# epam/ai-dial-rag

Measured on AMD Instinct MI355X. Metric: retrieval_qps_10Mx384, higher is better.
Workload: dtype f32 (int8 MFMA filter with exact integer dot products and a rigorous error margin, every candidate the margin cannot exclude re-scored in f64 with the reference formula)

## Files before the change

### ai-dial-rag_amd/csrc/vec_kernels_i8.h

```cpp
#pragma once
#include "vec_kernels_sieve.h"

#ifndef I8_ABL
#define I8_ABL 0
#endif

namespace mir {

typedef int __attribute__((ext_vector_type(4))) i32x4;

constexpr int kI8StatWords = 8;
constexpr int kI8MaxK = 16;
static_assert(kI8MaxK <= kSieveSampleMaxK, "the exact sample threshold evaluates k rows in one round");
constexpr int kI8Region = 32768;
constexpr int kI8WavePart = kI8Region / 8;
__device__ __forceinline__ void i8_margin_ab(float qn, float eq, const float *__restrict__ stats, float &A, float &B) {
    i8_margin_ab_decl(qn, eq, stats, A, B);
}
__device__ __forceinline__ float i8_margin_tile(bool l2, float A, float B, float e_t, float s_t, float sq) {
    const float m = fmaf(e_t, A, B) + 2.0f * s_t * sq;
    return l2 ? 2.0f * m : m;
}

__global__ __launch_bounds__(256) void i8_tile_scale_kernel(const float *__restrict__ src, int64_t n, int d, float4 *__restrict__ tparam) {
    __shared__ float red[4];
    const int64_t tile = blockIdx.x;
    const int64_t r0 = tile * kTileRows;
    const int64_t rows = n - r0 < kTileRows ? n - r0 : kTileRows;
    const float *p = src + r0 * (int64_t)d;
    float m = 0.f;
    for (int64_t i = threadIdx.x; i < rows * d; i += 256) m = fmaxf(m, fabsf(p[i]));
#pragma unroll
    for (int off = 32; off >= 1; off >>= 1) m = fmaxf(m, __shfl_xor(m, off, 64));
    if ((threadIdx.x & 63) == 0) red[threadIdx.x >> 6] = m;
    __syncthreads();
    if (threadIdx.x == 0) {
        m = fmaxf(fmaxf(red[0], red[1]), fmaxf(red[2], red[3]));
        const float st = m > 0.f ? m / 127.0f : 1.0f;
        tparam[tile] = make_float4(st, 0.f, 0.5f / st, 0.f);
    }
}
__global__ void i8_scale_kernel(float *__restrict__ stats, const float *__restrict__ max_norm) {
    stats[0] = max_norm[0];
    stats[7] = __builtin_inff();
}

__device__ __forceinline__ int i8_quant(float x, float inv) {
    const float r = rintf(x * inv);
    return (int)fminf(fmaxf(r, -127.0f), 127.0f);
}

__global__ __launch_bounds__(256) void pack_i8_kernel(const float *__restrict__ src, int64_t n, int d, int ks64, int64_t total_lanes,
                                                      const float4 *__restrict__ tparam, uint4 *__restrict__ dst) {
    const int64_t gid = (int64_t)blockIdx.x * 256 + threadIdx.x;
    if (gid >= total_lanes) return;
    const int lane = (int)(gid & 63);
    const int64_t blk = gid >> 6;
    const int nb = ks64 * 2;
    const int b = (int)(blk % nb);
    const int64_t tile = blk / nb;
    const int s = b >> 1, rh = b & 1;
    const int64_t row = tile * kTileRows + 16 * rh + (lane & 15);
    const int col0 = 64 * s + 16 * (lane >> 4);
    uint32_t w[4] = {0u, 0u, 0u, 0u};
    if (row < n) {
        const float inv = 1.0f / tparam[tile].x;
#pragma unroll
        for (int j = 0; j < 16; ++j) {
            const float x = col0 + j < d ? src[row * (int64_t)d + col0 + j] : 0.f;
            w[j >> 2] |= ((uint32_t)i8_quant(x, inv) & 0xffu) << (8 * (j & 3));
        }
    }
    dst[blk * 64 + lane] = make_uint4(w[0], w[1], w[2], w[3]);
}

__global__ __launch_bounds__(256) void i8_residual_kernel(const float *__restrict__ src, int64_t n, int d, const float *__restrict__ doc_sq,
                                                          float4 *__restrict__ tparam, float *__restrict__ stats) {
    const int lg = threadIdx.x & 15;
    const int64_t row = (int64_t)blockIdx.x * 16 + (threadIdx.x >> 4);
    double e2 = 0.0;
    if (row < n) {
        const float s = tparam[row / kTileRows].x;
        const float inv = 1.0f / s;
        for (int j = lg; j < d; j += 16) {
            const float x = src[row * (int64_t)d + j];
            const double r = (double)x - (double)s * (double)i8_quant(x, inv);
            e2 += r * r;
        }
    }
    e2 = group_sum<16>(e2);
    if (lg == 0 && row < n) {
        const float e = (float)sqrt(e2) * (1.0f + 1e-6f);
        atomicMax(reinterpret_cast<unsigned int *>(&tparam[row / kTileRows].y), __float_as_uint(e));
        const float a = doc_sq[row];
        const volatile float *vs = stats;
        if (e > vs[2]) atomicMax(reinterpret_cast<unsigned int *>(stats) + 2, __float_as_uint(e));
        if (a > vs[1]) atomicMax(reinterpret_cast<unsigned int *>(stats) + 1, __float_as_uint(a));
        if (a < vs[7]) atomicMin(reinterpret_cast<unsigned int *>(stats) + 7, __float_as_uint(a));
    }
}

__global__ __launch_bounds__(128) void i8_stage_record_kernel(const float *__restrict__ col, int64_t n_col, const float4 *__restrict__ tparam,
                                                              float *__restrict__ rec) {
    const int64_t stage = blockIdx.x;
    const int t = threadIdx.x;
    if (t >= 72) return;
    float v;
    if (t < 64) {
        const int64_t row = stage * 64 + t;
        v = row < n_col ? col[row] : 0.f;
    } else {
        v = reinterpret_cast<const float *>(tparam)[stage * 8 + (t - 64)];
    }
    rec[stage * 72 + t] = v;
}

__global__ __launch_bounds__(64) void prep_queries_i8_stats_kernel(const double *__restrict__ q, int b, int d, double *__restrict__ q_sq,
                                                                   double *__restrict__ q_norm, float *__restrict__ q_amax,
                                                                   unsigned long long *__restrict__ gthr, int gthr_words) {
    const int lane = threadIdx.x, blk = blockIdx.x;
    if (gthr && blk * 64 + lane < gthr_words) gthr[blk * 64 + lane] = 0;
    const int qi = blk;
    if (qi >= b) return;
    double s = 0.0;
    float m = 0.f;
    bool bad = false;
    for (int j = lane; j < d; j += 64) {
        const double x = q[(int64_t)qi * d + j];
        s += x * x;
        const float a = fabsf((float)x);
        bad |= !(a < __builtin_inff());
        m = fmaxf(m, a);
    }
    s = wave_sum(s);
#pragma unroll
    for (int off = 32; off >= 1; off >>= 1) m = fmaxf(m, __shfl_xor(m, off, 64));
    bad = __any(bad);
    if (lane == 0) {
        q_sq[qi] = s;
        q_norm[qi] = sqrt(s);
        q_amax[qi] = bad ? -1.0f : m;
    }
}
__global__ __launch_bounds__(64) void prep_queries_i8_quant_kernel(const double *__restrict__ q, int b, int d, int ks64, int ntiles16,
                                                                   const float *__restrict__ q_amax, uint4 *__restrict__ qfrag,
                                                                   double *__restrict__ q_err, float *__restrict__ q_scale) {
    const int lane = threadIdx.x, blk = blockIdx.x;
    if (blk < ntiles16 * ks64) {
        const int s = blk % ks64, w = blk / ks64;
        const int qi = 16 * w + (lane & 15);
        const int col0 = 64 * s + 16 * (lane >> 4);
        uint32_t wv[4] = {0u, 0u, 0u, 0u};
        const float m = qi < b ? q_amax[qi] : -1.0f;
        if (m >= 0.f) {
            const float inv = m > 0.f ? 127.0f / m : 1.0f;
#pragma unroll
            for (int j = 0; j < 16; ++j) {
                const float x = col0 + j < d ? (float)q[(int64_t)qi * d + col0 + j] : 0.f;
                wv[j >> 2] |= ((uint32_t)i8_quant(x, inv) & 0xffu) << (8 * (j & 3));
            }
        }
        qfrag[(int64_t)blk * 64 + lane] = make_uint4(wv[0], wv[1], wv[2], wv[3]);
    } else {
        const int qi = blk - ntiles16 * ks64;
        if (qi >= b) return;
        const float m = q_amax[qi];
        const bool ok = m >= 0.f;
        const float inv = m > 0.f ? 127.0f / m : 1.0f;
        const float sq = 1.0f / inv;
        double e2 = 0.0;
        for (int j = lane; j < d; j += 64) {
            const double x = q[(int64_t)qi * d + j];
            const double r = ok ? x - (double)sq * (double)i8_quant((float)x, inv) : x;
            e2 += r * r;
        }
        e2 = wave_sum(e2);
        if (lane == 0) {
            q_err[qi] = sqrt(e2);
            q_scale[qi] = sq;
        }
    }
}

__host__ __device__ constexpr int sieve_i8_stages(int nw) { return nw == 8 ? kSieveStages : 3; }
__host__ __device__ constexpr size_t sieve_i8_lds_bytes(int ks64, int nw) { return (size_t)sieve_i8_stages(nw) * (ks64 * 4 * 1024 + (64 + 8) * 4) + 64; }

template <int KS64, int KIND, bool SAMPLE, int QT, int NW>
__global__ __launch_bounds__(NW * 64, 2) void sieve_i8_kernel(const uint4 *__restrict__ docs, const float *__restrict__ aux,
                                                          const uint4 *__restrict__ qfrag, const double *__restrict__ q_norm,
                                                          const double *__restrict__ q_sq, const double *__restrict__ q_err,
                                                          const float *__restrict__ stats, const float *__restrict__ q_scale,
                                                          uint32_t n_rows, uint32_t stage0, uint32_t n_stages, int nq, int nan_guard,
                                                          const uint64_t *__restrict__ gthr, uint64_t *__restrict__ cand,
                                                          float *__restrict__ candv, uint32_t *__restrict__ ccount,
                                                          float *__restrict__ part_sample, unsigned long long *__restrict__ stat) {
    static_assert(KIND == SCAN_L2 || KIND == SCAN_IP || KIND == SCAN_COS, "scan kind");
    static_assert(QT == 1 || QT == 2 || QT == 4, "query tiles per wave");
    static_assert(NW == 8 || NW == 4, "waves per workgroup");
    constexpr int NS = sieve_i8_stages(NW);
    constexpr int APW = 64 / NW;
    constexpr int NB = KS64 * 2;
    constexpr int SB = NB * 2;
    constexpr int STAGE_U4 = SB * 64;
    constexpr int PPW = SB / NW;
    constexpr int PW = PPW + 1;
    constexpr int AS = 64 + 8;
    constexpr int D = NS - 1;
    constexpr int QPL = NW * 16 * QT;
    static_assert(SB % NW == 0, "sieve_i8: d padded to a multiple of 128");
    extern __shared__ __attribute__((aligned(16))) unsigned char smem[];
    uint4 *ring = reinterpret_cast<uint4 *>(smem);
    float *aux_lds = reinterpret_cast<float *>(smem + (size_t)NS * STAGE_U4 * 16);

    const int tid = threadIdx.x, lane = tid & 63, qc = lane & 15, jg = lane >> 4;
    const int wave8 = __builtin_amdgcn_readfirstlane(tid >> 6);
    const uint32_t G = gridDim.x;

    const float amin = KIND == SCAN_L2 ? stats[7] : 0.f;
    int qloc[QT];
    bool lane_live[QT];
    unsigned long long live_mask[QT];
    constexpr float L = KIND == SCAN_L2 ? 2.0f : 1.0f;
    const float ax_hi = KIND == SCAN_COS ? stats[6] : 1.0f;
    float tbc[QT];
    float sq[QT], mA[QT], mB[QT], P1[QT], A1[QT], guard[QT], best[QT];
    uint32_t brow[QT];
    i32x4 qh[QT][KS64];
    const bool active = nq > wave8 * QT * 16;
#pragma unroll
    for (int u = 0; u < QT; ++u) {
        const int t16 = wave8 * QT + u;
        qloc[u] = t16 * 16 + qc;
        lane_live[u] = qloc[u] < nq && (SAMPLE || query_filterable(KIND == SCAN_L2, q_norm[qloc[u]], stats[0]));
        live_mask[u] = __builtin_amdgcn_ballot_w64(lane_live[u]);
        sq[u] = 1.0f; mA[u] = 0.f; mB[u] = 0.f; P1[u] = -__builtin_inff(); A1[u] = 0.f; tbc[u] = -__builtin_inff();
        guard[u] = __builtin_inff(); best[u] = -__builtin_inff(); brow[u] = 0;
        if (lane_live[u]) {
            const float qn = (float)q_norm[qloc[u]] * (1.0f + 1e-6f);
            const float eq = (float)q_err[qloc[u]] * (1.0f + 1e-6f);
            const bool good = qn < __builtin_inff() && eq < __builtin_inff();
            sq[u] = q_scale[qloc[u]];
            if (good) i8_margin_ab(qn, eq, stats, mA[u], mB[u]);
            if (!SAMPLE) {
                const uint64_t key = gthr[qloc[u]];
                if (key != 0 && good) {
                    const float t = key_value(key);
                    float tb = t - 2e-6f * fabsf(t);
                    tbc[u] = tb;
                    if (KIND == SCAN_COS) tb = fminf(tb * stats[4], tb * stats[5]) - 1e-6f * fabsf(tb) * stats[5];
                    P1[u] = (tb + amin - L * mB[u]) / (L * sq[u]);
                    A1[u] = mA[u] / sq[u];
                    if (!(P1[u] == P1[u]) || !(A1[u] == A1[u])) { P1[u] = -__builtin_inff(); A1[u] = 0.f; tbc[u] = -__builtin_inff(); }
                }
            } else if (nan_guard) {
                const float qs = (float)q_sq[qloc[u]];
                guard[u] = qs - 1e-5f * fabsf(qs);
            }
        }
        const uint4 *qs = qfrag + (size_t)t16 * KS64 * 64 + lane;
#pragma unroll
        for (int s = 0; s < KS64; ++s) qh[u][s] = __builtin_bit_cast(i32x4, qs[s * 64]);
    }
    const uint32_t my_stages = blockIdx.x < n_stages ? (n_stages - blockIdx.x + G - 1) / G : 0;
    const uint32_t NG = my_stages;

    auto issue = [&](uint32_t g) {
        const uint32_t stage = stage0 + blockIdx.x + g * G;
        const uint4 *src = docs + (size_t)stage * STAGE_U4 + (wave8 * PPW) * 64 + lane;
        const uint32_t dst = __builtin_amdgcn_readfirstlane(lds_addr_of(ring) + ((g % NS) * STAGE_U4 + (wave8 * PPW) * 64) * 16);
#pragma unroll
        for (int i = 0; i < PPW; ++i) glds16_b128(src + i * 64, dst + i * 1024);
        {
            const uint32_t adst = __builtin_amdgcn_readfirstlane(lds_addr_of(aux_lds) + ((g % NS) * AS + wave8 * APW) * 4);
            const float *abase = aux + (size_t)stage * AS + wave8 * APW;
            if (lane < APW + (wave8 == NW - 1 ? 8 : 0)) glds4_b32_sv(abase, (uint32_t)lane * 4u, adst);
        }
    };
#pragma unroll
    for (int u = 0; u < QT; ++u)
#pragma unroll
        for (int s = 0; s < KS64; ++s) asm volatile("" : "+v"(qh[u][s]));
    asm volatile("s_waitcnt vmcnt(0)" ::: "memory");
    for (uint32_t g = 0; g < (uint32_t)D && g < NG; ++g) issue(g);

    auto wait_stage = [&](uint32_t g) {
        const uint32_t younger = (NG - 1 - g) < (uint32_t)(D - 1) ? (NG - 1 - g) : (uint32_t)(D - 1);
        if (younger == (uint32_t)(D - 1)) asm volatile("s_waitcnt vmcnt(%0)" ::"i"((D - 1) * PW) : "memory");
        else asm volatile("s_waitcnt vmcnt(0)" ::: "memory");
    };
    uint64_t *region = cand + ((size_t)blockIdx.x * NW + wave8) * kI8WavePart;
    float *regionv = candv + ((size_t)blockIdx.x * NW + wave8) * kI8WavePart;
    const unsigned long long lt_mask = (1ull << lane) - 1ull;
    uint32_t wcount = 0;

    auto filter = [&](int u, const i32x4 &c0, const i32x4 &c1, const float (&ax)[8], uint32_t t, const float4 &tp) {
        if (SAMPLE) {
            if (lane_live[u]) {
                const float vs = L * tp.x * sq[u], mg = i8_margin_tile(KIND == SCAN_L2, mA[u], mB[u], tp.y, tp.x, sq[u]) * ax_hi;
#pragma unroll
                for (int r = 0; r < 8; ++r) {
                    const float fi = (float)(r < 4 ? c0[r & 3] : c1[r & 3]);
                    const float w = KIND == SCAN_L2 ? fmaf(vs, fi, -ax[r]) : KIND == SCAN_COS ? vs * fi * ax[r] : vs * fi;
                    const uint32_t row = t * kTileRows + 4 * jg + 16 * (r >> 2) + (r & 3);
                    if (w + mg < guard[u] && w - mg > best[u] && row < n_rows) { best[u] = w - mg; brow[u] = row; }
                }
            }
            return;
        }
        const float x2 = fmaf(fmaf(-tp.y, A1[u], P1[u]), 2.0f * tp.z, -4.0f);
        const int ib = (int)__builtin_amdgcn_fmed3f(floorf(x2), -2.0e9f, 2.0e9f);
        const int m0 = max(max(c0[0], c0[1]), c0[2]), m1 = max(max(c0[3], c1[0]), c1[1]);
        const int m = max(max(max(c1[2], c1[3]), m0), m1);
        if ((__builtin_amdgcn_ballot_w64(m >= ib) & live_mask[u]) == 0ull) return;
        asm volatile("" : "+s"(t));
        const float vs = L * tp.x * sq[u];
        float bound = (fmaf(-tp.y, A1[u], P1[u]) - 2.0f * tp.x) * (L * sq[u]) - amin;
        if (KIND == SCAN_COS) bound = tbc[u] - i8_margin_tile(false, mA[u], mB[u], tp.y, tp.x, sq[u]) * ax_hi;
        const float bound_w = bound - 4e-6f * (fabsf(bound) + amin);
        float v[8];
#pragma unroll
        for (int r = 0; r < 8; ++r) {
            const float fi = (float)(r < 4 ? c0[r & 3] : c1[r & 3]);
            v[r] = KIND == SCAN_L2 ? fmaf(vs, fi, -ax[r]) : KIND == SCAN_COS ? vs * fi * ax[r] : vs * fi;
        }
        uint32_t pm = 0;
#pragma unroll
        for (int r = 0; r < 8; ++r) pm |= (uint32_t)(!(v[r] < bound_w)) << r;
        if (!lane_live[u]) pm = 0;
        if (!__any(pm != 0)) return;
        const uint32_t row0 = t * kTileRows + 4 * jg;
        if (t * kTileRows + kTileRows > n_rows) {
#pragma unroll
            for (int r = 0; r < 8; ++r)
                if (row0 + 16 * (r >> 2) + (r & 3) >= n_rows) pm &= ~(1u << r);
        }
        while (__any(pm != 0)) {
            const bool has = pm != 0;
            const int r = has ? __builtin_ctz(pm) : 0;
            const unsigned long long bal = __ballot(has);
            const uint32_t slot = wcount + (uint32_t)__popcll(bal & lt_mask);
            wcount += (uint32_t)__popcll(bal);
            float vr = v[0];
#pragma unroll
            for (int i = 1; i < 8; ++i) vr = r == i ? v[i] : vr;
            if (has && slot < (uint32_t)kI8WavePart) {
                region[slot] = ((uint64_t)(uint32_t)qloc[u] << 32) | (uint64_t)(row0 + 16 * (r >> 2) + (r & 3));
                regionv[slot] = vr;
            }
            pm &= pm - 1;
        }
    };

    i32x4 p0[QT], p1[QT];
#pragma unroll
    for (int u = 0; u < QT; ++u) { p0[u] = i32x4{0, 0, 0, 0}; p1[u] = i32x4{0, 0, 0, 0}; }
    float pax[8] = {};
    float4 ptp = make_float4(1.f, 0.f, 0.5f, 0.f);
    uint32_t pt = 0;
    bool have_prev = false;
    for (uint32_t g = 0; g < my_stages; ++g) {
        const uint32_t stage = stage0 + blockIdx.x + g * G;
#if !(I8_ABL & 4)
        wait_stage(g);
#endif
#if !(I8_ABL & 2)
        __builtin_amdgcn_s_barrier();
#endif
        if (!active) {
            if (g + D < NG) issue(g + D);
            continue;
        }
#pragma unroll
        for (int sub = 0; sub < 2; ++sub) {
            const uint4 *st = ring + (size_t)(g % NS) * STAGE_U4 + sub * (NB * 64) + lane;
            constexpr int PF = QT == 4 ? 1 : (2 < KS64 ? 2 : KS64 - 1);
            uint4 f0[PF + 1], f1[PF + 1];
#pragma unroll
            for (int i = 0; i < PF; ++i) { f0[i] = st[(2 * i + 0) * 64]; f1[i] = st[(2 * i + 1) * 64]; }
            const float4 ctp = *reinterpret_cast<const float4 *>(aux_lds + (g % NS) * AS + 64 + 4 * sub);
            float cax[8] = {};
            if (KIND != SCAN_IP) {
                const float4 a0 = *reinterpret_cast<const float4 *>(aux_lds + (g % NS) * AS + 32 * sub + 4 * jg);
                const float4 a1 = *reinterpret_cast<const float4 *>(aux_lds + (g % NS) * AS + 32 * sub + 16 + 4 * jg);
                cax[0] = a0.x; cax[1] = a0.y; cax[2] = a0.z; cax[3] = a0.w;
                cax[4] = a1.x; cax[5] = a1.y; cax[6] = a1.z; cax[7] = a1.w;
            }
            i32x4 c0[QT], c1[QT];
#pragma unroll
            for (int u = 0; u < QT; ++u) { c0[u] = i32x4{0, 0, 0, 0}; c1[u] = i32x4{0, 0, 0, 0}; }
#pragma unroll
            for (int s = 0; s < KS64; ++s) {
                if (s + PF < KS64) {
                    f0[(s + PF) % (PF + 1)] = st[(2 * (s + PF) + 0) * 64];
                    f1[(s + PF) % (PF + 1)] = st[(2 * (s + PF) + 1) * 64];
                }
                __builtin_amdgcn_sched_barrier(0);
#pragma unroll
                for (int u = 0; u < QT; ++u) {
                    c0[u] = __builtin_amdgcn_mfma_i32_16x16x64_i8(__builtin_bit_cast(i32x4, f0[s % (PF + 1)]), qh[u][s], c0[u], 0, 0, 0);
                    c1[u] = __builtin_amdgcn_mfma_i32_16x16x64_i8(__builtin_bit_cast(i32x4, f1[s % (PF + 1)]), qh[u][s], c1[u], 0, 0, 0);
                }
                if (sub == 0 && s == 0) {
                    __builtin_amdgcn_sched_barrier(0);
#if !(I8_ABL & 4)
                    if (g + D < NG) issue(g + D);
#endif
                }
#pragma unroll
                for (int u = 0; u < QT; ++u)
                    if (s == 1 + u && s < KS64 && have_prev) {
                        __builtin_amdgcn_sched_barrier(0);
#if I8_ABL & 1
                        if (g == 0xffffff)
#endif
                        filter(u, p0[u], p1[u], pax, pt, ptp);
                    }
            }
            if (KS64 < QT + 1 && have_prev) {
#pragma unroll
                for (int u = KS64 - 1; u < QT; ++u) filter(u, p0[u], p1[u], pax, pt, ptp);
            }
#pragma unroll
            for (int u = 0; u < QT; ++u) { p0[u] = c0[u]; p1[u] = c1[u]; }
#pragma unroll
            for (int i = 0; i < 8; ++i) pax[i] = cax[i];
            ptp = ctp;
            pt = stage * 2 + sub;
            have_prev = true;
        }
    }
    if (have_prev) {
#pragma unroll
        for (int u = 0; u < QT; ++u) filter(u, p0[u], p1[u], pax, pt, ptp);
    }
    if (SAMPLE) {
        uint32_t *part_row = reinterpret_cast<uint32_t *>(part_sample + (size_t)gridDim.x * QPL * 2);
#pragma unroll
        for (int u = 0; u < QT; ++u) {
            const float o = __shfl_xor(best[u], 16, 64);
            const uint32_t orow = (uint32_t)__shfl_xor((int)brow[u], 16, 64);
            const bool other = o > best[u];
            const float b2 = other ? o : best[u];
            const size_t at = ((size_t)blockIdx.x * QPL + qloc[u]) * 2 + (jg >> 1);
            if (lane_live[u] && (jg == 0 || jg == 2)) {
                part_sample[at] = b2;
                part_row[at] = other ? orow : brow[u];
            }
        }
        return;
    }
    if (lane == 0) {
        ccount[(size_t)blockIdx.x * NW + wave8] = wcount;
        if (stat && wcount) atomicAdd(stat, (unsigned long long)wcount);
    }
}

__global__ __launch_bounds__(256) void sieve_scatter_i8_kernel(SieveScatterArgs a) {
    __shared__ uint32_t s_cnt[256], s_base[256];
    const int tid = threadIdx.x;
    const int part = blockIdx.x;
    uint32_t cnt = a.ccount[part];
    s_cnt[tid] = 0;
    __syncthreads();
    if (cnt > (uint32_t)kI8WavePart) {
        for (int i = tid; i < a.nq; i += 256) a.l.over[a.q0 + i] = 1;
        cnt = kI8WavePart;
    }
    const uint64_t *region = a.cand + (size_t)part * kI8WavePart;
    const float *regionv = a.candv + (size_t)part * kI8WavePart;
    for (uint32_t e = tid; e < cnt; e += 256) atomicAdd(&s_cnt[(int)(region[e] >> 32) & 255], 1u);
    __syncthreads();
    {
        const uint32_t c = s_cnt[tid];
        s_base[tid] = c ? atomicAdd(&a.l.count[(size_t)(a.q0 + tid) * kSieveCountStride], c) : 0u;
        s_cnt[tid] = 0;
    }
    __syncthreads();
    for (uint32_t e = tid; e < cnt; e += 256) {
        const uint64_t key = region[e];
        const int ql = (int)(key >> 32) & 255, qi = a.q0 + ql;
        const uint32_t slot = s_base[ql] + atomicAdd(&s_cnt[ql], 1u);
        if (slot < (uint32_t)kSieveQueryCap) {
            a.l.row[(size_t)qi * kSieveQueryCap + slot] = (uint32_t)key;
            a.l.rv[(size_t)qi * kSieveQueryCap + slot] = regionv[e];
        } else {
            a.l.over[qi] = 1;
        }
    }
}

}
```

Measured before the change: 254,400.

## Restructure int8 MFMA loop to filter one query tile behind with double-buffered accumulators

The per-stage loop changes from processing two row-halves with QT query accumulators each to iterating over 2*QT query blocks. Each block uses one pair of double-buffered accumulators, and the filter test for the previous block is interleaved inside the MFMA chain. All K fragments of a half-stage are loaded into registers up front, and the next half is prefetched during the last block, which cuts accumulator register pressure. The floor-and-clamp conversion is also replaced with a single v_cvt_flr_i32_f32 instruction. The change risks different scheduling, higher fragment register use, and changed tail handling for the last filter.

```diff
diff --git a/ai-dial-rag_amd/csrc/vec_kernels_i8.h b/ai-dial-rag_amd/csrc/vec_kernels_i8.h
--- a/ai-dial-rag_amd/csrc/vec_kernels_i8.h
+++ b/ai-dial-rag_amd/csrc/vec_kernels_i8.h
@@ -293,7 +293,7 @@
     const unsigned long long lt_mask = (1ull << lane) - 1ull;
     uint32_t wcount = 0;
 
-    auto filter = [&](int u, const i32x4 &c0, const i32x4 &c1, const float (&ax)[8], uint32_t t, const float4 &tp) {
+    auto test = [&](int u, const i32x4 &c0, const i32x4 &c1, uint32_t t, const float4 &tp, const float (&ax)[8]) __attribute__((always_inline)) {
         if (SAMPLE) {
             if (lane_live[u]) {
                 const float vs = L * tp.x * sq[u], mg = i8_margin_tile(KIND == SCAN_L2, mA[u], mB[u], tp.y, tp.x, sq[u]) * ax_hi;
@@ -308,7 +308,8 @@
             return;
         }
         const float x2 = fmaf(fmaf(-tp.y, A1[u], P1[u]), 2.0f * tp.z, -4.0f);
-        const int ib = (int)__builtin_amdgcn_fmed3f(floorf(x2), -2.0e9f, 2.0e9f);
+        int ib;
+        asm("v_cvt_flr_i32_f32 %0, %1" : "=v"(ib) : "v"(x2));
         const int m0 = max(max(c0[0], c0[1]), c0[2]), m1 = max(max(c0[3], c1[0]), c1[1]);
         const int m = max(max(max(c1[2], c1[3]), m0), m1);
         if ((__builtin_amdgcn_ballot_w64(m >= ib) & live_mask[u]) == 0ull) return;
@@ -350,14 +351,20 @@
             pm &= pm - 1;
         }
     };
-
-    i32x4 p0[QT], p1[QT];
-#pragma unroll
-    for (int u = 0; u < QT; ++u) { p0[u] = i32x4{0, 0, 0, 0}; p1[u] = i32x4{0, 0, 0, 0}; }
-    float pax[8] = {};
-    float4 ptp = make_float4(1.f, 0.f, 0.5f, 0.f);
-    uint32_t pt = 0;
-    bool have_prev = false;
+#if I8_ABL & 1
+#define I8_TEST(...) do { if (n_rows == 0xfffffff1u) test(__VA_ARGS__); } while (0)
+#else
+#define I8_TEST(...) test(__VA_ARGS__)
+#endif
+
+    constexpr int K = 2 * KS64;
+    constexpr int BPS = 2 * QT;
+    i32x4 ca[2], cb[2];
+#pragma unroll
+    for (int i = 0; i < 2; ++i) { ca[i] = i32x4{0, 0, 0, 0}; cb[i] = i32x4{0, 0, 0, 0}; }
+    float4 tp = make_float4(1.f, 0.f, 0.5f, 0.f);
+    float ax[8] = {};
+    uint32_t dt = 0;
     for (uint32_t g = 0; g < my_stages; ++g) {
         const uint32_t stage = stage0 + blockIdx.x + g * G;
 #if !(I8_ABL & 4)
@@ -370,69 +377,73 @@
             if (g + D < NG) issue(g + D);
             continue;
         }
-#pragma unroll
-        for (int sub = 0; sub < 2; ++sub) {
-            const uint4 *st = ring + (size_t)(g % NS) * STAGE_U4 + sub * (NB * 64) + lane;
-            constexpr int PF = QT == 4 ? 1 : (2 < KS64 ? 2 : KS64 - 1);
-            uint4 f0[PF + 1], f1[PF + 1];
-#pragma unroll
-            for (int i = 0; i < PF; ++i) { f0[i] = st[(2 * i + 0) * 64]; f1[i] = st[(2 * i + 1) * 64]; }
-            const float4 ctp = *reinterpret_cast<const float4 *>(aux_lds + (g % NS) * AS + 64 + 4 * sub);
-            float cax[8] = {};
-            if (KIND != SCAN_IP) {
-                const float4 a0 = *reinterpret_cast<const float4 *>(aux_lds + (g % NS) * AS + 32 * sub + 4 * jg);
-                const float4 a1 = *reinterpret_cast<const float4 *>(aux_lds + (g % NS) * AS + 32 * sub + 16 + 4 * jg);
-                cax[0] = a0.x; cax[1] = a0.y; cax[2] = a0.z; cax[3] = a0.w;
-                cax[4] = a1.x; cax[5] = a1.y; cax[6] = a1.z; cax[7] = a1.w;
-            }
-            i32x4 c0[QT], c1[QT];
-#pragma unroll
-            for (int u = 0; u < QT; ++u) { c0[u] = i32x4{0, 0, 0, 0}; c1[u] = i32x4{0, 0, 0, 0}; }
-#pragma unroll
-            for (int s = 0; s < KS64; ++s) {
-                if (s + PF < KS64) {
-                    f0[(s + PF) % (PF + 1)] = st[(2 * (s + PF) + 0) * 64];
-                    f1[(s + PF) % (PF + 1)] = st[(2 * (s + PF) + 1) * 64];
-                }
-                __builtin_amdgcn_sched_barrier(0);
-#pragma unroll
-                for (int u = 0; u < QT; ++u) {
-                    c0[u] = __builtin_amdgcn_mfma_i32_16x16x64_i8(__builtin_bit_cast(i32x4, f0[s % (PF + 1)]), qh[u][s], c0[u], 0, 0, 0);
-                    c1[u] = __builtin_amdgcn_mfma_i32_16x16x64_i8(__builtin_bit_cast(i32x4, f1[s % (PF + 1)]), qh[u][s], c1[u], 0, 0, 0);
-                }
-                if (sub == 0 && s == 0) {
+        const uint4 *st = ring + (size_t)(g % NS) * STAGE_U4 + lane;
+        const float *rec = aux_lds + (g % NS) * AS;
+        uint4 F[K];
+#pragma unroll
+        for (int j = 0; j < K; ++j) {
+            F[j] = st[j * 64];
+            __builtin_amdgcn_sched_barrier(0);
+        }
+#pragma unroll
+        for (int b = 0; b < BPS; ++b) {
+            const int u = b % QT, P = b & 1, Pp = P ^ 1;
+            const int pu = (b + QT - 1) % QT;
+            const uint32_t pt = b == 0 ? dt : stage * 2 + (uint32_t)((b - 1) / QT);
+            const bool pf = !(I8_ABL & 8) && b == QT - 1;
+#if I8_ABL & 8
+            if (b == QT) {
+#pragma unroll
+                for (int j = 0; j < K; ++j) { F[j] = st[(K + j) * 64]; __builtin_amdgcn_sched_barrier(0); }
+            }
+#endif
+            ca[P] = i32x4{0, 0, 0, 0};
+            cb[P] = i32x4{0, 0, 0, 0};
+#pragma unroll
+            for (int j = 0; j < K; ++j) {
+                if (j & 1) cb[P] = __builtin_amdgcn_mfma_i32_16x16x64_i8(__builtin_bit_cast(i32x4, F[j]), qh[u][j >> 1], cb[P], 0, 0, 0);
+                else ca[P] = __builtin_amdgcn_mfma_i32_16x16x64_i8(__builtin_bit_cast(i32x4, F[j]), qh[u][j >> 1], ca[P], 0, 0, 0);
+                if (pf && j > 0) { F[j - 1] = st[(K + j - 1) * 64]; __builtin_amdgcn_sched_barrier(0); }
+                if (!(I8_ABL & 8) && b == QT && j == 0) F[K - 1] = st[(2 * K - 1) * 64];
+                if (j == 1) {
                     __builtin_amdgcn_sched_barrier(0);
+                    if (b == 0) {
+                        if (g != 0) I8_TEST(pu, ca[Pp], cb[Pp], pt, tp, ax);
+                    } else {
+                        I8_TEST(pu, ca[Pp], cb[Pp], pt, tp, ax);
+                    }
+                    __builtin_amdgcn_sched_barrier(0);
+                    if (b % QT == 0) {
+                        tp = *reinterpret_cast<const float4 *>(rec + 64 + 4 * (b / QT));
+                        if (KIND != SCAN_IP) {
+                            const float4 a0 = *reinterpret_cast<const float4 *>(rec + 32 * (b / QT) + 4 * jg);
+                            const float4 a1 = *reinterpret_cast<const float4 *>(rec + 32 * (b / QT) + 16 + 4 * jg);
+                            ax[0] = a0.x; ax[1] = a0.y; ax[2] = a0.z; ax[3] = a0.w;
+                            ax[4] = a1.x; ax[5] = a1.y; ax[6] = a1.z; ax[7] = a1.w;
+                        }
+                        __builtin_amdgcn_sched_barrier(0);
+                    }
 #if !(I8_ABL & 4)
-                    if (g + D < NG) issue(g + D);
+                    if (b == 0) {
+                        if (g + D < NG) issue(g + D);
+                        __builtin_amdgcn_sched_barrier(0);
+                    }
 #endif
                 }
-#pragma unroll
-                for (int u = 0; u < QT; ++u)
-                    if (s == 1 + u && s < KS64 && have_prev) {
-                        __builtin_amdgcn_sched_barrier(0);
-#if I8_ABL & 1
-                        if (g == 0xffffff)
-#endif
-                        filter(u, p0[u], p1[u], pax, pt, ptp);
-                    }
-            }
-            if (KS64 < QT + 1 && have_prev) {
-#pragma unroll
-                for (int u = KS64 - 1; u < QT; ++u) filter(u, p0[u], p1[u], pax, pt, ptp);
-            }
-#pragma unroll
-            for (int u = 0; u < QT; ++u) { p0[u] = c0[u]; p1[u] = c1[u]; }
-#pragma unroll
-            for (int i = 0; i < 8; ++i) pax[i] = cax[i];
-            ptp = ctp;
-            pt = stage * 2 + sub;
-            have_prev = true;
-        }
-    }
-    if (have_prev) {
-#pragma unroll
-        for (int u = 0; u < QT; ++u) filter(u, p0[u], p1[u], pax, pt, ptp);
-    }
+            }
+        }
+        dt = stage * 2 + 1;
+        asm volatile("" : "+v"(tp.x), "+v"(tp.y), "+v"(tp.z));
+        if (KIND != SCAN_IP) {
+#pragma unroll
+            for (int i = 0; i < 8; ++i) asm volatile("" : "+v"(ax[i]));
+        }
+    }
+    if (my_stages != 0 && active) {
+        constexpr int Pl = (BPS - 1) & 1;
+        I8_TEST(QT - 1, ca[Pl], cb[Pl], dt, tp, ax);
+    }
+#undef I8_TEST
     if (SAMPLE) {
         uint32_t *part_row = reinterpret_cast<uint32_t *>(part_sample + (size_t)gridDim.x * QPL * 2);
 #pragma unroll
```

New measurement: 229,900. -9.6%, worse.
